# fujii-team/deComP

Hardware: AMD Instinct MI355X
Metric: nmf_mu_iterations_per_s (higher is better)
Workload: dtype f32; 1 GPU; nmf_mu l2 no-mask Y=65536x4096 k=256 fp32 (BASELINE configs[1]); rows_per_gpu=65536, parallelism=rows sharded x1, 1 all-reduce/step, loop=single-GPU dcp_nmf_mu_f32

## Files before the change

decomp_amd/_hip.py:

```python
import ctypes
import os
import threading

_HERE = os.path.dirname(os.path.abspath(__file__))
LIB_PATH = os.path.join(_HERE, 'lib', 'libdecomp_hip.so')

OK = 0
ERR_NAMES = {-1: 'DCP_ERR_INVALID', -2: 'DCP_ERR_HIP', -3: 'DCP_ERR_NOMEM',
             -4: 'DCP_ERR_INTERNAL', -5: 'DCP_ERR_UNSUPPORTED', -6: 'DCP_ERR_REF_TYPEERROR',
             -7: 'DCP_ERR_COMM'}
LIK_L2, LIK_KL, LIK_BETA = 0, 1, 2
PROF_NLABELS = 10
PROF_XUPDATE, PROF_STATS = 2, 4
LASSO_ISTA, LASSO_ACC_ISTA, LASSO_FISTA, LASSO_CD = 0, 1, 2, 3
LASSO_PARALLEL_CD, LASSO_ADMM = 4, 5
LASSO_OMP = 6
LASSO_POSITIVE = 0x100
ERR_REF_TYPEERROR = -6
ERR_COMM = -7
COMM_ID_BYTES = 128
ALLREDUCE_FN = ctypes.CFUNCTYPE(ctypes.c_int, ctypes.c_void_p, ctypes.c_int64, ctypes.c_int, ctypes.c_void_p, ctypes.c_void_p)

_c_int, _c_i64, _c_vp = ctypes.c_int, ctypes.c_int64, ctypes.c_void_p
_c_f32, _c_f64 = ctypes.c_float, ctypes.c_double
# ... 6 lines not shown
_P_INT, _P_F64 = _P(_c_int), _P(_c_f64)
_NFK = [_c_i64] * 3
_TM = [_c_i64] * 5 + [_c_int]
_TM_MC = [_c_i64] * 6 + [_c_int]
_MASKED = [_c_vp] * 3 + [_c_int, _c_vp, _c_vp] + _NFK

_FAMILIES = [
    ('dcp_create', None, [_P(_c_vp), _c_int]),
    ('dcp_destroy', None, [_c_vp]),
    ('dcp_set_stream', None, [_c_vp, _c_vp]),
    ('dcp_last_error_string', None, [_c_vp], ctypes.c_char_p),
    ('dcp_build_info', None, [], ctypes.c_char_p),
    ('dcp_comm_unique_id', None, [_c_vp, _c_i64]),
    ('dcp_comm_init', None, [_c_vp, _c_vp, _c_int, _c_int]),
    ('dcp_comm_destroy', None, [_c_vp]),
    ('dcp_comm_set_external', None, [_c_vp] * 3 + [_c_int, _c_int]),
    ('dcp_memcpy', None, [_c_vp] * 3 + [_c_i64]),
    ('dcp_comm_info', None, [_c_vp, _P_INT, _P_INT]),
    ('dcp_comm_allreduce_sum', _REALS, [_c_vp, _c_vp, _c_i64]),
    ('dcp_profile_enable', None, [_c_vp, _c_int]),
    ('dcp_profile_reset', None, [_c_vp]),
    ('dcp_profile_select', None, [_c_vp, ctypes.c_uint]),
    ('dcp_profile_read', None, [_c_vp, _c_int, _P_F64, _P(_c_i64)]),
    ('dcp_profile_label_name', None, [_c_int], ctypes.c_char_p),
    ('dcp_l2_normalize', _ALL, [_c_vp, _c_vp, _c_i64, _c_i64, _c_int]),
    ('dcp_l2_normalize_diff', _REALS, [_c_vp] * 4 + [_c_i64, _c_i64, _c_int, _P_F64]),
    ('dcp_count_negative', _REALS, [_c_vp, _c_vp, _c_i64, _P(_c_i64)]),
    ('dcp_gershgorin', _ALL, [_c_vp, _c_vp, _c_i64, _c_i64, _c_vp]),
    ('dcp_inv', _ALL, [_c_vp, _c_vp, _c_i64, _c_i64, _c_vp]),
    ('dcp_mu_quotient', _REALS, [_c_vp] * 4 + [_c_i64, _c_i64, _c_vp]),
    ('dcp_axpby', _REALS, [_c_vp, _c_i64, _c_f64, _c_vp, _c_f64, _c_vp]),
    ('dcp_gemm', _ALL, [_c_vp, _c_int] + [_c_vp] * 3 + _NFK + [_c_int, _c_int]),
    ('dcp_gemm_bf16x6', ('f32',), [_c_vp, _c_int] + [_c_vp] * 3 + _NFK + [_c_int]),
    ('dcp_set_f32_product_mode', None, [_c_vp, _c_int]),
    ('dcp_debug_tn_plain', None, [_c_int]),
    ('dcp_debug_gemm_route', None, [_c_int, _c_int] + [_c_i64] * 4 + [_c_int] * 5 + [_c_vp]),
    ('dcp_calib_read', ('f32',), [_c_vp, _c_vp, _c_i64, _c_i64, _c_int, _c_vp]),
    ('dcp_gather_rows_bytes', None, [_c_vp] * 3 + [_c_i64, _c_i64, _c_vp]),
    ('dcp_scatter_rows_bytes', None, [_c_vp] * 3 + [_c_i64, _c_i64, _c_vp]),
    ('dcp_dict_prefetch_rows_bytes', None, [_c_vp] * 3 + [_c_i64, _c_i64, _c_vp]),
    ('dcp_gather_rows', _ALL, [_c_vp] * 3 + [_c_i64, _c_i64, _c_vp]),
    ('dcp_nmf_mu', _REALS, [_c_vp] * 5 + _NFK + [_c_int, _REAL, _c_int, _P_INT, _P_REAL, _P_REAL]),
    ('dcp_nmf_mu_sharded', _REALS, [_c_vp] * 5 + _NFK + [_c_int, _REAL, _c_int, _P_INT, _P_REAL]),
    ('dcp_nmf_hals', _REALS, [_c_vp] * 4 + _NFK + [_REAL, _c_int, _P_INT, _P_REAL, _P_REAL]),
    ('dcp_nmf_hals_sharded', _REALS, [_c_vp] * 4 + _NFK + [_REAL, _c_int, _P_INT, _P_REAL]),
    ('dcp_nmf_emhals', _REALS, [_c_vp] * 5 + _NFK + [_REAL, _c_int, _P_INT, _P_REAL, _P_REAL]),
    ('dcp_nmf_emhals_sharded', _REALS, [_c_vp] * 5 + _NFK + [_REAL, _c_int, _P_INT, _P_REAL]),
    ('dcp_nmf_impute', _REALS, [_c_vp] * 5 + _NFK + [_c_vp]),
    ('dcp_nmf_hals_stats', _REALS, [_c_vp] * 5 + _NFK + [_c_vp]),
    ('dcp_nmf_hals_update', _REALS, [_c_vp] * 5 + _NFK + [_c_vp, _c_vp]),
    ('dcp_nn_cd_sweep', _REALS, [_c_vp] * 5 + [_c_i64, _c_i64, _c_int]),
    ('dcp_nmf_mu_stats_width', None, [_c_i64, _c_i64, _c_int, _c_int], _c_i64),
    ('dcp_nmf_mu_stats', _REALS, [_c_vp] * 6 + _NFK + [_c_int, _c_vp]),
    ('dcp_nmf_mask_bits_words', None, [_c_i64, _c_i64], _c_i64),
    ('dcp_nmf_mask_prepare', _REALS, [_c_vp] * 3 + [_c_i64, _c_i64, _c_vp, _c_vp, _P_INT]),
    ('dcp_nmf_mu_stats_prepared', _REALS, [_c_vp] * 7 + _NFK + [_c_int, _c_vp]),
    ('dcp_nmf_mu_update', _REALS, [_c_vp] * 4 + [_c_i64, _c_i64, _c_int, _c_int, _c_vp, _c_vp]),
    ('dcp_nmf_grads', _REALS, [_c_vp] * 5 + _NFK + [_c_int, _c_int, _c_vp, _c_vp]),
    ('dcp_nmf_grad_x', _REALS, [_c_vp] * 5 + _NFK + [_c_int, _c_vp, _c_vp]),
    ('dcp_nmf_gauss_logp', _REALS, [_c_vp] * 5 + _NFK + [_c_f64, _P_F64]),
    ('dcp_set_nmf_beta', None, [_c_vp, _c_f64]),
    ('dcp_set_nmf_penalty', None, [_c_vp, _c_f64, _c_f64]),
    ('dcp_nmf_beta_divergence', _REALS, [_c_vp] * 5 + _NFK + [_P_F64]),
    ('dcp_nmf_apply', _REALS, [_c_vp] * 4 + [_c_f64, _c_vp, _c_i64, _c_i64, _P_F64]),
    ('dcp_nmf_residual', _REALS, [_c_vp] * 5 + _NFK + [_P_F64]),
    ('dcp_lasso', _ALL, _MASKED + [_c_f64, _c_f64, _c_int, _c_int, _c_int, _P_INT]),
# ... 107 lines not shown
```

decomp_amd/csrc/gemm.hpp:

```cpp
#pragma once
#include <type_traits>

#include "epilogue.hpp"
#include "gemm_generic.hpp"
#include "gemm_mfma_bf16x6.hpp"
#include "gemm_mfma_f32.hpp"
#include "gemm_mfma_f64.hpp"
#include "reduce.hpp"
#include "scalar.hpp"

namespace dcp {

enum GemmForm { FORM_NT = 0, FORM_NN = 1, FORM_TN = 2 };
enum TileSel { TILE_AUTO = 0, TILE_LARGE = 1, TILE_SMALL = 2, TILE_HUGE = 3, TILE_SMALL_DEEP = 4, TILE_MID = 5 };

template <class T>
struct GemmArgs {
    const T* A = nullptr;
    long lda = 0;
    const T* B = nullptr;
    long ldb = 0;
    const T* B2 = nullptr;
    long ldb2 = 0;
    int n_b1 = 0;
// ... 459 lines not shown
enum { X6_NONE = -1, X6_LARGE = 0, X6_HUGE = 1 };
constexpr int kX6HugeTnMinK = 1024;

template <class T>
inline bool x6_huge_tn_shape(const GemmArgs<T>& a, int n1, int klen) {
    return std::is_same<T, float>::value && a.A2 == nullptr && a.M > 0 && a.N > 0 && a.K > 0 &&
           a.M % X6Huge::BM == 0 && n1 % X6Huge::BN == 0 && (a.N - n1) % X6Huge::BN == 0 && klen >= kX6HugeTnMinK &&
           pick_tier<FORM_TN>(a.M, a.N, a.K, a.tile, true, true) == TIER_LARGE;
}

template <class T>
inline bool plan_splits_x6_tn(GemmArgs<T>& a, int n1, int max_splits) {
    if (a.M <= 0 || a.N <= 0 || a.K <= 0 || a.M % X6Huge::BM || n1 % X6Huge::BN || (a.N - n1) % X6Huge::BN)
        return false;
    const long tiles = (long)(a.M / X6Huge::BM) * (n1 / X6Huge::BN + (a.N - n1) / X6Huge::BN);
    const long kblocks = ceil_div(a.K, 16);
    long smax = kblocks / 32;
    if (smax < 1) smax = 1;
    if (smax > max_splits) smax = max_splits;
    long s = 256 / tiles;
    if (s > smax) s = smax;
    if (s < 1) s = 1;
    const int klen = (int)(((kblocks + s - 1) / s) * 16);
    if (!x6_huge_tn_shape(a, n1, klen)) return false;
    a.split_planned = true;
    a.klen = klen;
    a.ksplits = ceil_div(a.K, klen);
    return true;
}

template <int FORM>
inline int x6_tier(const GemmArgs<float>& a) {
    if (FORM == FORM_NN) return X6_NONE;
    const int tier = pick_tier<FORM>(a.M, a.N, a.K, a.tile, a.split_planned, true);
    const GemmProblem p = fill_problem<FORM>(a);
    if (FORM == FORM_NT && tier == TIER_HUGE && x6_eligible<X6Huge>(p)) return X6_HUGE;
    if (FORM == FORM_TN && tier == TIER_LARGE && x6_huge_tn_shape(a, a.B2 != nullptr ? a.n_b1 : a.N, a.ksplits > 1 ? a.klen : a.K) &&
        x6_eligible<X6Huge>(p))
        return X6_HUGE;
    if ((tier == TIER_LARGE || (FORM == FORM_NT && (tier == TIER_MID || tier == TIER_HUGE))) &&
        x6_eligible<X6Large>(p))
        return X6_LARGE;
    return X6_NONE;
}

template <int FORM, class Epi>
inline hipError_t gemm_bf16x6(hipStream_t stream, const GemmArgs<float>& a, const Epi& epi) {
    constexpr int AL = (FORM == FORM_TN) ? XMAJOR : KMAJOR;
    constexpr int BL = (FORM == FORM_NT) ? KMAJOR : XMAJOR;
    if constexpr (FORM == FORM_NN) {
        return hipErrorInvalidValue;
    } else {
        const int t = x6_tier<FORM>(a);
        if (t == X6_HUGE) return launch_gemm_bf16x6<X6Huge, AL, BL, Epi>(stream, fill_problem<FORM>(a), epi);
        if (t == X6_LARGE) return launch_gemm_bf16x6<X6Large, AL, BL, Epi>(stream, fill_problem<FORM>(a), epi);
        return hipErrorInvalidValue;
    }
}

}
```

decomp_amd/csrc/gemm_mfma_bf16x6.hpp:

```cpp
#pragma once
#include "gemm_mfma_f32.hpp"
#include <type_traits>

namespace dcp {

typedef __bf16 x6_bf16x4 __attribute__((ext_vector_type(4)));
typedef __bf16 x6_bf16x8 __attribute__((ext_vector_type(8)));

template <int BM_, int BN_, int WM_, int WN_, int MINW_, int STAGES_>
struct X6Cfg {
    static constexpr int BM = BM_, BN = BN_, BK = 16, WM = WM_, WN = WN_, MINW = MINW_;
    static constexpr int NWAVES = (BM_ / WM_) * (BN_ / WN_);
    static constexpr int NTHREADS = 64 * NWAVES;
    static constexpr int STAGES = STAGES_;
};
typedef X6Cfg<256, 256, 64, 64, 1, 3> X6Huge;
typedef X6Cfg<128, 128, 64, 64, 2, 2> X6Large;

template <int ROWS>
struct X6Panel {
    static constexpr int PLANE_BYTES = ROWS * 32;
    static constexpr int BYTES = 3 * PLANE_BYTES;
};

__device__ __forceinline__ int x6_chunk(int r, int q) { return r * 32 + ((q ^ ((r >> 3) & 1)) << 4); }

__device__ __forceinline__ void x6_split(f32x4 a, x6_bf16x4& h, x6_bf16x4& m, x6_bf16x4& l) {
    h = __builtin_convertvector(a, x6_bf16x4);
    const f32x4 r1 = a - __builtin_convertvector(h, f32x4);
    m = __builtin_convertvector(r1, x6_bf16x4);
    const f32x4 r2 = r1 - __builtin_convertvector(m, f32x4);
    l = __builtin_convertvector(r2, x6_bf16x4);
}

template <int LAY, int ROWS, int NT, int G>
__device__ __forceinline__ void x6_gload(f32x4 (&r)[G], const float* __restrict__ p, long ld, int row0, int k0,
                                         int tid) {
    static_assert(G * NT * 4 == ROWS * 16, "panel must be a whole number of 4-value groups per thread");
#pragma unroll
    for (int i = 0; i < G; ++i) {
        const int idx = tid + i * NT;
        if (LAY == KMAJOR) {
            const int row = idx >> 2, kq = idx & 3;
            r[i] = *reinterpret_cast<const f32x4*>(p + (long)(row0 + row) * ld + (k0 + 4 * kq));
        } else {
            const int g = idx % (ROWS / 4), k = idx / (ROWS / 4);
            r[i] = *reinterpret_cast<const f32x4*>(p + (long)(k0 + k) * ld + (row0 + 4 * g));
        }
    }
}

template <int ROWS>
__device__ __forceinline__ int x6_granule(int k, int g) {
    static_assert(ROWS >= 128, "the XOR swizzle needs 32 granules per k row");
    return k * (ROWS * 2) + ((g ^ ((k & 3) << 3)) << 3);
}

template <int LAY, int ROWS, int NT, int G>
__device__ __forceinline__ void x6_lds_store(char* s, const f32x4 (&r)[G], int tid) {
#pragma unroll
    for (int i = 0; i < G; ++i) {
        const int idx = tid + i * NT;
        int off;
        if (LAY == KMAJOR) {
            const int row = idx >> 2, kq = idx & 3;
            off = x6_chunk(row, kq >> 1) + ((kq & 1) << 3);
        } else {
            off = x6_granule<ROWS>(idx / (ROWS / 4), idx % (ROWS / 4));
        }
        x6_bf16x4 h, m, l;
        x6_split(r[i], h, m, l);
        *reinterpret_cast<x6_bf16x4*>(s + off) = h;
        *reinterpret_cast<x6_bf16x4*>(s + X6Panel<ROWS>::PLANE_BYTES + off) = m;
        *reinterpret_cast<x6_bf16x4*>(s + 2 * X6Panel<ROWS>::PLANE_BYTES + off) = l;
    }
}

template <int LAY, int ROWS>
__device__ __forceinline__ int x6_frag_off(int r0, int lane) {
    const int l31 = lane & 31, h = lane >> 5;
    if (LAY == KMAJOR) return x6_chunk(r0 + l31, h);
    const int q = (lane >> 2) & 3, pq = lane & 3, gh = (lane >> 4) & 1;
    return x6_granule<ROWS>(8 * h + q, (r0 >> 2) + 4 * gh + pq);
}

template <int LAY, int ROWS>
__device__ __forceinline__ x6_bf16x8 x6_frag(const char* plane, int off) {
    if (LAY == KMAJOR) return *reinterpret_cast<const x6_bf16x8*>(plane + off);
    typedef short s16x4 __attribute__((ext_vector_type(4)));
    typedef __attribute__((address_space(3))) s16x4 lds_s16x4;
    const s16x4 lo = __builtin_amdgcn_ds_read_tr16_b64_v4i16((lds_s16x4*)(plane + off));
    const s16x4 hi = __builtin_amdgcn_ds_read_tr16_b64_v4i16((lds_s16x4*)(plane + off + 4 * ROWS * 2));
    return __builtin_bit_cast(x6_bf16x8, __builtin_shufflevector(lo, hi, 0, 1, 2, 3, 4, 5, 6, 7));
}

template <class E, class = void>
struct epi_den_tail { static constexpr bool value = false; };
template <class E>
struct epi_den_tail<E, decltype((void)E::kDenTail)> { static constexpr bool value = E::kDenTail; };

typedef float x6_f32x2 __attribute__((ext_vector_type(2)));

__device__ __forceinline__ int x6_den_xoff(int r, int q) { return r * 16 + ((q ^ ((r >> 2) & 3)) << 2); }

template <class Epi>
__device__ __forceinline__ void x6_den_tail(f32x16 (&num)[2][2], const Epi& epi, char* smem, int m0, int n0, int tid) {
    constexpr int XS = 128 * 16 * 4;
    constexpr int GS = 16 * 256 * 4;
    constexpr int DBUF = XS + GS;
    const int lane = tid & 63, wave = tid >> 6;
    const int wm = wave >> 2, wn = wave & 3;
    const int l31 = lane & 31, h = lane >> 5;
    const int nkd = epi.depth >> 4;

    const int pr = tid >> 3, k2 = tid & 7;
    const float* xsrc = epi.cur + (long)(m0 + (pr >> 5) * 64 + (pr & 31)) * epi.ld_cur + 2 * k2;
    const int xdst = (x6_den_xoff(pr, k2 >> 1) + 2 * (k2 & 1)) * 4;
// ... 120 lines not shown
    int mt, nt;
    if (p.mt_fast) {
        mt = t % p.tiles_m;
        nt = t / p.tiles_m;
    } else {
        nt = t % p.tiles_n;
        mt = t / p.tiles_n;
    }
    const int m0 = mt * BM;
    const int kbeg = split * p.klen;
    const int kend = min(p.K, kbeg + p.klen);
    const float* Bp = p.B;
    long ldb = p.ldb;
    int nB0 = nt * BN;
    int n0 = nB0;
    if (nt >= p.tiles_n1) {
        Bp = p.B2;
        ldb = p.ldb2;
        nB0 = (nt - p.tiles_n1) * BN;
        n0 = p.n_b1 + nB0;
    }

    f32x16 acc[TM][TN];
#pragma unroll
    for (int i = 0; i < TM; ++i)
#pragma unroll
        for (int j = 0; j < TN; ++j)
#pragma unroll
            for (int r = 0; r < 16; ++r) acc[i][j][r] = 0.0f;

    static_assert(TM == 2, "one panel's staging per 32-row A block");
    constexpr int STAGES = Cfg::STAGES;
    static_assert(STAGES == 2 || STAGES == 3, "two buffers and a boundary barrier, or a ring of three");
    f32x4 ra[GA], rb[GB];
    const int nkb = (kend - kbeg) / BK;
    if (nkb > 0) {
        x6_gload<ALAY, BM, NT>(ra, p.A, p.lda, m0, kbeg, tid);
        x6_gload<BLAY, BN, NT>(rb, Bp, ldb, nB0, kbeg, tid);
        x6_lds_store<ALAY, BM, NT>(x6_smem, ra, tid);
        x6_lds_store<BLAY, BN, NT>(x6_smem + X6Panel<BM>::BYTES, rb, tid);
        const int k1 = kbeg + min(1, nkb - 1) * BK;
        x6_gload<ALAY, BM, NT>(ra, p.A, p.lda, m0, k1, tid);
        x6_gload<BLAY, BN, NT>(rb, Bp, ldb, nB0, k1, tid);
        if constexpr (STAGES == 3) {
            x6_lds_store<ALAY, BM, NT>(x6_smem + BUF, ra, tid);
            x6_lds_store<BLAY, BN, NT>(x6_smem + BUF + X6Panel<BM>::BYTES, rb, tid);
            const int k2 = kbeg + min(2, nkb - 1) * BK;
            x6_gload<ALAY, BM, NT>(ra, p.A, p.lda, m0, k2, tid);
            x6_gload<BLAY, BN, NT>(rb, Bp, ldb, nB0, k2, tid);
        }
    }
    __syncthreads();

    int aoff[TM], boff[TN];
#pragma unroll
    for (int i = 0; i < TM; ++i) aoff[i] = x6_frag_off<ALAY, BM>(wm * WM + i * 32, lane);
#pragma unroll
    for (int j = 0; j < TN; ++j) boff[j] = x6_frag_off<BLAY, BN>(wn * WN + j * 32, lane);

    constexpr int STAGE_AFTER = 2;
    auto kblock = [&](int cur, int nxt_off, int knext, auto stage_tag, auto bar_tag) {
        constexpr bool STAGE = decltype(stage_tag)::value;
        constexpr bool BAR = decltype(bar_tag)::value;
        const char* sA = x6_smem + cur;
        const char* sB = sA + X6Panel<BM>::BYTES;
        char* nxt = x6_smem + nxt_off;
        x6_bf16x8 fb[3][TN];
#pragma unroll
        for (int pl = 0; pl < 3; ++pl)
#pragma unroll
            for (int j = 0; j < TN; ++j) fb[pl][j] = x6_frag<BLAY, BN>(sB + pl * PB, boff[j]);
        constexpr int TA[6] = {2, 0, 1, 1, 0, 0};
        constexpr int TB[6] = {0, 2, 1, 0, 1, 0};
        auto group = [&](auto i_tag) {
            constexpr int i = decltype(i_tag)::value;
            x6_bf16x8 fa[3];
#pragma unroll
            for (int pl = 0; pl < 3; ++pl) fa[pl] = x6_frag<ALAY, BM>(sA + pl * PA, aoff[i]);
            if constexpr (BAR && i == 1) {
                __builtin_amdgcn_sched_barrier(0);
                __syncthreads();
                __builtin_amdgcn_sched_barrier(0);
            }
            auto mfmas = [&](int t0, int t1) {
#pragma unroll
                for (int tt = t0; tt < t1; ++tt)
#pragma unroll
                    for (int j = 0; j < TN; ++j)
                        acc[i][j] =
                            __builtin_amdgcn_mfma_f32_32x32x16_bf16(fa[TA[tt]], fb[TB[tt]][j], acc[i][j], 0, 0, 0);
            };
            if constexpr (STAGE) {
                mfmas(0, STAGE_AFTER);
                __builtin_amdgcn_sched_barrier(0);
                if constexpr (i == 0) {
                    x6_lds_store<ALAY, BM, NT>(nxt, ra, tid);
                    x6_gload<ALAY, BM, NT>(ra, p.A, p.lda, m0, knext, tid);
                } else {
                    x6_lds_store<BLAY, BN, NT>(nxt + X6Panel<BM>::BYTES, rb, tid);
                    x6_gload<BLAY, BN, NT>(rb, Bp, ldb, nB0, knext, tid);
                }
                __builtin_amdgcn_sched_barrier(0);
                mfmas(STAGE_AFTER, 6);
            } else {
                mfmas(0, 6);
            }
            __builtin_amdgcn_sched_barrier(0);
        };
        group(std::integral_constant<int, 0>{});
        group(std::integral_constant<int, 1>{});
    };
    if constexpr (STAGES == 2) {
        for (int kb = 0; kb + 1 < nkb; ++kb) {
            const int cur = (kb & 1) * BUF;
            kblock(cur, cur ^ BUF, kbeg + min(kb + 2, nkb - 1) * BK, std::true_type{}, std::false_type{});
            __syncthreads();
        }
        if (nkb > 0) kblock(((nkb - 1) & 1) * BUF, 0, 0, std::false_type{}, std::false_type{});
    } else {
        int b0 = 0, b1 = BUF, b2 = 2 * BUF;
        for (int kb = 0; kb + 2 < nkb; ++kb) {
            kblock(b0, b2, kbeg + min(kb + 3, nkb - 1) * BK, std::true_type{}, std::true_type{});
            const int t0 = b0;
            b0 = b1;
            b1 = b2;
            b2 = t0;
        }
        if (nkb > 1) kblock(b0, 0, 0, std::false_type{}, std::true_type{});
        if (nkb > 0) kblock(nkb > 1 ? b1 : b0, 0, 0, std::false_type{}, std::false_type{});
    }

    if constexpr (epi_den_tail<Epi>::value) {
        static_assert(BM == 256 && BN == 256 && NT == 1024 && STAGES == 3 && ALAY == KMAJOR && BLAY == KMAJOR,
                      "the denominator tail is laid out for the 256 x 256 NT tile");
        x6_den_tail(acc, epi, x6_smem, m0, n0, tid);
    } else if constexpr (epi_vec4<Epi>::value) {
        const int tq = l31 & 3, col0 = (l31 & ~3);
#pragma unroll
        for (int i = 0; i < TM; ++i)
#pragma unroll
            for (int j = 0; j < TN; ++j)
#pragma unroll
                for (int g = 0; g < 4; ++g) {
                    f32x4 x;
#pragma unroll
                    for (int e = 0; e < 4; ++e) x[e] = acc[i][j][4 * g + e];
                    const f32x4 y = quad_transpose(x, tq);
                    epi.vec4(m0 + wm * WM + i * 32 + 8 * g + 4 * h + tq, n0 + wn * WN + j * 32 + col0, y, split);
                }
    } else {
#pragma unroll
        for (int i = 0; i < TM; ++i)
#pragma unroll
            for (int j = 0; j < TN; ++j) {
                const int col = n0 + wn * WN + j * 32 + l31;
#pragma unroll
                for (int r = 0; r < 16; ++r) {
                    const int row = m0 + wm * WM + i * 32 + (r & 3) + 8 * (r >> 2) + 4 * h;
                    epi(row, col, acc[i][j][r], split);
                }
            }
    }
}

template <class Epi>
inline bool x6_epi_ok(const Epi& epi) {
    if constexpr (epi_vec4<Epi>::value) return epi.vec_ok();
    else return true;
}

template <class Cfg>
inline bool x6_eligible(const GemmProblem& p) {
    auto al16 = [](const void* q) { return (reinterpret_cast<uintptr_t>(q) & 15) == 0; };
    const int n1 = p.B2 != nullptr ? p.n_b1 : p.N;
    bool ok = p.M > 0 && p.N > 0 && p.K > 0 && (p.M % Cfg::BM) == 0 && (n1 % Cfg::BN) == 0 &&
              ((p.N - n1) % Cfg::BN) == 0 && (p.K % 16) == 0 && p.A2 == nullptr && (p.lda % 4) == 0 &&
              (p.ldb % 4) == 0 && al16(p.A) && al16(p.B);
    if (p.B2 != nullptr) ok = ok && (p.ldb2 % 4) == 0 && al16(p.B2);
    if (p.ksplits > 1) ok = ok && (p.klen % 16) == 0 && p.klen > 0;
    return ok;
}

template <class Cfg, int ALAY, int BLAY, class Epi>
inline hipError_t launch_gemm_bf16x6(hipStream_t stream, GemmProblem p, const Epi& epi) {
    if (!x6_eligible<Cfg>(p) || !x6_epi_ok(epi)) return hipErrorInvalidValue;
    if constexpr (epi_den_tail<Epi>::value) {
        if (p.ksplits > 1 || p.B2 != nullptr || epi.depth < 48 || (epi.depth % 16) != 0) return hipErrorInvalidValue;
    }
    if (p.B2 == nullptr) p.n_b1 = p.N;
    p.m_a1 = p.M;
    p.tiles_m1 = p.tiles_m = p.M / Cfg::BM;
    p.tiles_n1 = p.n_b1 / Cfg::BN;
    p.tiles_n = p.tiles_n1 + (p.N - p.n_b1) / Cfg::BN;
    if (p.ksplits < 1) p.ksplits = 1;
    if (p.ksplits == 1) p.klen = p.K;
    p.vec_epi = epi_vec4<Epi>::value ? 1 : 0;
    p.al_mask = 0;
    const int grid = p.tiles_m * p.tiles_n * p.ksplits;
    if (grid <= 0) return hipSuccess;
    constexpr int lds_bytes = Cfg::STAGES * (X6Panel<Cfg::BM>::BYTES + X6Panel<Cfg::BN>::BYTES);
    const void* fn = reinterpret_cast<const void*>(&gemm_bf16x6_kernel<Cfg, ALAY, BLAY, Epi>);
    if constexpr (lds_bytes > 65536) {
        static DynLdsRaised raised;
        std::atomic<bool>& done = raised.on_current_device();
        if (!done) {
            hipError_t e = hipFuncSetAttribute(fn, hipFuncAttributeMaxDynamicSharedMemorySize, lds_bytes);
            if (e != hipSuccess) return e;
            done = true;
        }
    }
    hipLaunchKernelGGL((gemm_bf16x6_kernel<Cfg, ALAY, BLAY, Epi>), dim3(grid), dim3(Cfg::NTHREADS), lds_bytes,
                       stream, p, epi);
    return hipGetLastError();
}

}
```

decomp_amd/csrc/util.hip:

```cpp
#include "abi.hpp"
#include "comm.hpp"
#include "gemm.hpp"
#include "handle.hpp"
#include "kernels_small.hpp"
#include <new>

#define DCP_STR2(x) #x
#define DCP_STR(x) DCP_STR2(x)

using namespace dcp;

namespace {

template <class T>
int l2_normalize_api(dcp_handle* h, T* U, int64_t K, int64_t F, int strict) {
    if (!h) return DCP_ERR_INVALID;
    if (!U) return fail(h, DCP_ERR_INVALID, "null array pointer");
    if (K < 0 || F < 0) return fail(h, DCP_ERR_INVALID, "negative size");
    if (K == 0 || F == 0) return DCP_OK;
    DCP_HIP_OK(h, hipSetDevice(h->device));
    hipLaunchKernelGGL((row_normalize_kernel<T>), dim3((unsigned)K), dim3(256), 0, h->stream,
                       (const T*)U, (long)F, (long)F, strict, (const T*)nullptr, 0L, U, (long)F,
                       (real_t<T>*)nullptr);
    DCP_HIP_OK(h, hipGetLastError());
// ... 473 lines not shown
        h->prof_cnt[i] = 0;
    }
    return DCP_OK;
}

int dcp_profile_read(dcp_handle* h, int label, double* total_ms, int64_t* count) {
    if (!h) return DCP_ERR_INVALID;
    if (label < 0 || label >= DCP_PROF_NLABELS || !total_ms || !count)
        return fail(h, DCP_ERR_INVALID, "bad profile label or null output");
    DCP_TRY(prof_fold(h));
    *total_ms = h->prof_ms[label];
    *count = h->prof_cnt[label];
    return DCP_OK;
}

const char* dcp_profile_label_name(int label) {
    static const char* names[DCP_PROF_NLABELS] = {"gram",  "x_neg",     "x_update", "forward", "stats",
                                                  "stats_sum", "d_update", "d_norm",  "misc", "exchange"};
    return (label >= 0 && label < DCP_PROF_NLABELS) ? names[label] : "?";
}

const char* dcp_last_error_string(dcp_handle* h) { return h ? h->err.c_str() : "null handle"; }

const char* dcp_build_info(void) {
    return "libdecomp_hip: gfx950, fp32 MFMA 32x32x2 + fp64 MFMA 16x16x4 GEMM cores, HIP " DCP_STR(HIP_VERSION_MAJOR) "." DCP_STR(HIP_VERSION_MINOR);
}

int dcp_count_negative_f32(dcp_handle* h, const float* x, int64_t n, int64_t* count) {
    return count_negative_api<float>(h, x, n, count);
}
int dcp_count_negative_f64(dcp_handle* h, const double* x, int64_t n, int64_t* count) {
    return count_negative_api<double>(h, x, n, count);
}
int dcp_gemm_bf16x6_f32(dcp_handle* h, int form, const float* A, const float* B, float* C, int64_t M, int64_t N,
                        int64_t K, int ksplits) {
    if (!h) return DCP_ERR_INVALID;
    if (!A || !B || !C) return fail(h, DCP_ERR_INVALID, "null array pointer");
    if (M <= 0 || N <= 0 || K <= 0 || M > INT32_MAX || N > INT32_MAX || K > INT32_MAX)
        return fail(h, DCP_ERR_INVALID, "bad sizes");
    if (form != FORM_NT && form != FORM_TN) return fail(h, DCP_ERR_INVALID, "bf16x6: form must be 0 (NT) or 2 (TN)");
    DCP_HIP_OK(h, hipSetDevice(h->device));
    GemmArgs<float> a;
    a.A = A; a.B = B; a.M = (int)M; a.N = (int)N; a.K = (int)K;
    a.lda = (form == FORM_TN) ? M : K;
    a.ldb = (form == FORM_NT) ? K : N;
    float* slabs = nullptr;
    if (ksplits > 1) {
        const long kblocks = (K + 15) / 16;
        const long s = ksplits > kblocks ? kblocks : ksplits;
        a.klen = (int)(((kblocks + s - 1) / s) * 16);
        a.ksplits = (int)((K + a.klen - 1) / a.klen);
        a.split_planned = true;
        DCP_TRY(ws_lay_out(h, [&](WsLayout& w) { w.take(slabs, (size_t)a.ksplits * M * N); }));
    }
    const bool ok = (form == FORM_NT) ? x6_tier<FORM_NT>(a) != X6_NONE : x6_tier<FORM_TN>(a) != X6_NONE;
    if (!ok) return fail(h, DCP_ERR_INVALID, "bf16x6: no split-bf16 kernel for this shape (tiles, alignment)");
    hipError_t e;
    if (slabs) {
        EpiSlab<float> epi{slabs, (long)N, (long)M * N};
        e = (form == FORM_NT) ? gemm_bf16x6<FORM_NT>(h->stream, a, epi) : gemm_bf16x6<FORM_TN>(h->stream, a, epi);
        if (e != hipSuccess) return fail(h, DCP_ERR_HIP, hipGetErrorString(e));
        launch_reduce_slabs_scalar<float>(h->stream, slabs, (long)(M * N), a.ksplits, (long)(M * N), C);
        DCP_HIP_OK(h, hipGetLastError());
    } else {
        EpiStore<float> epi{C, (long)N};
        e = (form == FORM_NT) ? gemm_bf16x6<FORM_NT>(h->stream, a, epi) : gemm_bf16x6<FORM_TN>(h->stream, a, epi);
        if (e != hipSuccess) return fail(h, DCP_ERR_HIP, hipGetErrorString(e));
    }
    return DCP_OK;
}
int dcp_set_f32_product_mode(dcp_handle* h, int mode) {
    if (!h) return DCP_ERR_INVALID;
    const int prev = h->f32_product_mode;
    if (mode > 1) return fail(h, DCP_ERR_INVALID, "f32 product mode must be 0 (bf16x6) or 1 (fp32)");
    if (mode >= 0) h->f32_product_mode = mode;
    return prev;
}

int dcp_dict_prefetch_rows_bytes(dcp_handle* h, const void* in, const int64_t* index, int64_t rows,
                                 int64_t row_bytes, void* out) {
    if (!h) return DCP_ERR_INVALID;
    if (rows < 0 || row_bytes < 0) return dcp::fail(h, DCP_ERR_INVALID, "negative size");
    if (rows > 0 && row_bytes > 0 && (!in || !index || !out)) return dcp::fail(h, DCP_ERR_INVALID, "null pointer");
    h->pf_in = in;
    h->pf_index = index;
    h->pf_out = out;
    h->pf_rows = rows;
    h->pf_row_bytes = row_bytes;
    return DCP_OK;
}

int dcp_gather_rows_bytes(dcp_handle* h, const void* in, const int64_t* index, int64_t rows,
                          int64_t row_bytes, void* out) {
    if (h && !index) return dcp::fail(h, DCP_ERR_INVALID, "null index");
    return move_rows(h, in, index, out, nullptr, rows, row_bytes);
}

int dcp_scatter_rows_bytes(dcp_handle* h, const void* in, const int64_t* index, int64_t rows,
                           int64_t row_bytes, void* out) {
    if (h && !index) return dcp::fail(h, DCP_ERR_INVALID, "null index");
    return move_rows(h, in, nullptr, out, index, rows, row_bytes);
}

// ... 22 lines not shown
```

include/decomp_hip.h:

```cpp
#ifndef DECOMP_HIP_H
#define DECOMP_HIP_H

#include <stdint.h>

#ifdef __cplusplus
extern "C" {
#endif

typedef struct dcp_handle dcp_handle;

enum {
    DCP_OK = 0,
    DCP_ERR_INVALID = -1,
    DCP_ERR_HIP = -2,
    DCP_ERR_NOMEM = -3,
    DCP_ERR_INTERNAL = -4,
    DCP_ERR_UNSUPPORTED = -5,
    DCP_ERR_REF_TYPEERROR = -6,
    DCP_ERR_COMM = -7
};

enum { DCP_LIK_L2 = 0, DCP_LIK_KL = 1, DCP_LIK_BETA = 2 };

enum { DCP_LASSO_ISTA = 0, DCP_LASSO_ACC_ISTA = 1, DCP_LASSO_FISTA = 2, DCP_LASSO_CD = 3,
// ... 36 lines not shown
int dcp_profile_reset(dcp_handle* h);
int dcp_profile_read(dcp_handle* h, int label, double* total_ms, int64_t* count);
const char* dcp_profile_label_name(int label);

int dcp_l2_normalize_f32(dcp_handle* h, float* U, int64_t K, int64_t F, int strict);
int dcp_l2_normalize_f64(dcp_handle* h, double* U, int64_t K, int64_t F, int strict);
int dcp_l2_normalize_c64(dcp_handle* h, void* U, int64_t K, int64_t F, int strict);
int dcp_l2_normalize_c128(dcp_handle* h, void* U, int64_t K, int64_t F, int strict);

int dcp_count_negative_f32(dcp_handle* h, const float* x, int64_t n, int64_t* count);
int dcp_count_negative_f64(dcp_handle* h, const double* x, int64_t n, int64_t* count);

int dcp_gershgorin_f32(dcp_handle* h, const float* X, int64_t batch, int64_t n, float* out);
int dcp_gershgorin_f64(dcp_handle* h, const double* X, int64_t batch, int64_t n, double* out);
int dcp_gershgorin_c64(dcp_handle* h, const void* X, int64_t batch, int64_t n, float* out);
int dcp_gershgorin_c128(dcp_handle* h, const void* X, int64_t batch, int64_t n, double* out);

int dcp_inv_f32(dcp_handle* h, const float* X, int64_t batch, int64_t n, float* out);
int dcp_inv_f64(dcp_handle* h, const double* X, int64_t batch, int64_t n, double* out);
int dcp_inv_c64(dcp_handle* h, const void* X, int64_t batch, int64_t n, void* out);
int dcp_inv_c128(dcp_handle* h, const void* X, int64_t batch, int64_t n, void* out);

int dcp_gemm_f32(dcp_handle* h, int form, const float* A, const float* B, float* C,
                 int64_t M, int64_t N, int64_t K, int ksplits, int tile);
int dcp_gemm_f64(dcp_handle* h, int form, const double* A, const double* B, double* C,
                 int64_t M, int64_t N, int64_t K, int ksplits, int tile);
int dcp_gemm_c64(dcp_handle* h, int form, const void* A, const void* B, void* C,
                 int64_t M, int64_t N, int64_t K, int ksplits, int tile);
int dcp_gemm_c128(dcp_handle* h, int form, const void* A, const void* B, void* C,
                  int64_t M, int64_t N, int64_t K, int ksplits, int tile);

int dcp_gemm_bf16x6_f32(dcp_handle* h, int form, const float* A, const float* B, float* C,
                        int64_t M, int64_t N, int64_t K, int ksplits);

int dcp_set_f32_product_mode(dcp_handle* h, int mode);

int dcp_debug_tn_plain(int on);

int dcp_debug_gemm_route(int dtype, int form, int64_t M, int64_t N, int64_t K, int64_t n_b1, int tile, int flags,
                         int target_wgs, int max_splits, int min_blocks, int32_t* out);

int dcp_calib_read_f32(dcp_handle* h, const float* p, int64_t rows, int64_t cols, int pattern,
                       float* out);

int dcp_nmf_mu_f32(dcp_handle* h, const float* Y, const float* mask, float* X, float* D,
                   int64_t N, int64_t F, int64_t K, int likelihood, float tol, int maxiter,
                   int* it_out, float* last_maxdiff, float* resid_trace);
int dcp_nmf_mu_f64(dcp_handle* h, const double* Y, const double* mask, double* X, double* D,
                   int64_t N, int64_t F, int64_t K, int likelihood, double tol, int maxiter,
                   int* it_out, double* last_maxdiff, double* resid_trace);

int dcp_nmf_hals_f32(dcp_handle* h, const float* Y, float* X, float* D, int64_t N, int64_t F, int64_t K,
                     float tol, int maxiter, int* it_out, float* last_maxdiff, float* resid_trace);
int dcp_nmf_hals_f64(dcp_handle* h, const double* Y, double* X, double* D, int64_t N, int64_t F, int64_t K,
                     double tol, int maxiter, int* it_out, double* last_maxdiff, double* resid_trace);
int dcp_nmf_hals_sharded_f32(dcp_handle* h, const float* Y, float* X, float* D, int64_t N, int64_t F, int64_t K,
                             float tol, int maxiter, int* it_out, float* last_maxdiff);
int dcp_nmf_hals_sharded_f64(dcp_handle* h, const double* Y, double* X, double* D, int64_t N, int64_t F, int64_t K,
                             double tol, int maxiter, int* it_out, double* last_maxdiff);
int dcp_nmf_hals_stats_f32(dcp_handle* h, const float* Y, const float* X, float* X_out, const float* D, int64_t N,
                           int64_t F, int64_t K, float* stats);
int dcp_nmf_hals_stats_f64(dcp_handle* h, const double* Y, const double* X, double* X_out, const double* D,
                           int64_t N, int64_t F, int64_t K, double* stats);
int dcp_nmf_hals_update_f32(dcp_handle* h, const float* stats, const float* D, float* D_new, float* X, int64_t N,
                            int64_t F, int64_t K, float* maxdiff_dev, float* maxdiff_next);
int dcp_nmf_hals_update_f64(dcp_handle* h, const double* stats, const double* D, double* D_new, double* X,
// ... 385 lines not shown
```

Baseline: 690.1 iterations/s.

## Preload bf16x6 LDS fragments across k-blocks and use scalar-base global loads

For the three-stage bf16x6 MFMA GEMM, the main loop now reads the next k-block's A/B fragments from LDS in small pieces between MFMA groups and moves the in-block barrier to sit between them. This is meant to hide LDS read latency behind matrix math instead of reloading all fragments at the start of each block. Global loads now use a scalar base pointer plus 32-bit per-lane offsets to cut address arithmetic, with an eligibility check that the offsets fit in 32 bits. It also adds a segmented-B API entry, a tier query helper and optional s_memtime timing stamps behind a compile flag, and it raises register pressure by keeping fragments live across blocks.

```diff
diff --git a/decomp_amd/_hip.py b/decomp_amd/_hip.py
--- a/decomp_amd/_hip.py
+++ b/decomp_amd/_hip.py
@@ -62,6 +62,8 @@
     ('dcp_axpby', _REALS, [_c_vp, _c_i64, _c_f64, _c_vp, _c_f64, _c_vp]),
     ('dcp_gemm', _ALL, [_c_vp, _c_int] + [_c_vp] * 3 + _NFK + [_c_int, _c_int]),
     ('dcp_gemm_bf16x6', ('f32',), [_c_vp, _c_int] + [_c_vp] * 3 + _NFK + [_c_int]),
+    ('dcp_gemm_bf16x6_seg', ('f32',), [_c_vp, _c_int] + [_c_vp] * 4 + [_c_i64] * 4 + [_c_int]),
+    ('dcp_gemm_bf16x6_tier', None, [_c_int] + [_c_i64] * 4 + [_c_int]),
     ('dcp_set_f32_product_mode', None, [_c_vp, _c_int]),
     ('dcp_debug_tn_plain', None, [_c_int]),
     ('dcp_debug_gemm_route', None, [_c_int, _c_int] + [_c_i64] * 4 + [_c_int] * 5 + [_c_vp]),
diff --git a/decomp_amd/csrc/gemm.hpp b/decomp_amd/csrc/gemm.hpp
--- a/decomp_amd/csrc/gemm.hpp
+++ b/decomp_amd/csrc/gemm.hpp
@@ -515,14 +515,15 @@
 template <int FORM>
 inline int x6_tier(const GemmArgs<float>& a) {
     if (FORM == FORM_NN) return X6_NONE;
+    constexpr int AL = (FORM == FORM_TN) ? XMAJOR : KMAJOR, BL = (FORM == FORM_NT) ? KMAJOR : XMAJOR;
     const int tier = pick_tier<FORM>(a.M, a.N, a.K, a.tile, a.split_planned, true);
     const GemmProblem p = fill_problem<FORM>(a);
-    if (FORM == FORM_NT && tier == TIER_HUGE && x6_eligible<X6Huge>(p)) return X6_HUGE;
+    if (FORM == FORM_NT && tier == TIER_HUGE && x6_eligible<X6Huge, AL, BL>(p)) return X6_HUGE;
     if (FORM == FORM_TN && tier == TIER_LARGE && x6_huge_tn_shape(a, a.B2 != nullptr ? a.n_b1 : a.N, a.ksplits > 1 ? a.klen : a.K) &&
-        x6_eligible<X6Huge>(p))
+        x6_eligible<X6Huge, AL, BL>(p))
         return X6_HUGE;
     if ((tier == TIER_LARGE || (FORM == FORM_NT && (tier == TIER_MID || tier == TIER_HUGE))) &&
-        x6_eligible<X6Large>(p))
+        x6_eligible<X6Large, AL, BL>(p))
         return X6_LARGE;
     return X6_NONE;
 }
diff --git a/decomp_amd/csrc/gemm_mfma_bf16x6.hpp b/decomp_amd/csrc/gemm_mfma_bf16x6.hpp
--- a/decomp_amd/csrc/gemm_mfma_bf16x6.hpp
+++ b/decomp_amd/csrc/gemm_mfma_bf16x6.hpp
@@ -3,6 +3,16 @@
 #include <type_traits>
 
 namespace dcp {
+
+#ifdef DCP_X6_STAMPS
+static __device__ unsigned long long x6_stamp_buf[16 * 8];
+#define X6_STAMP(t)                                                                         \
+    do {                                                                                    \
+        __builtin_amdgcn_sched_barrier(0);                                                  \
+        asm volatile("s_memtime %0\n\ts_waitcnt lgkmcnt(0)" : "=s"(t) : : "memory");        \
+        __builtin_amdgcn_sched_barrier(0);                                                  \
+    } while (0)
+#endif
 
 typedef __bf16 x6_bf16x4 __attribute__((ext_vector_type(4)));
 typedef __bf16 x6_bf16x8 __attribute__((ext_vector_type(8)));
@@ -33,20 +43,37 @@
     l = __builtin_convertvector(r2, x6_bf16x4);
 }
 
-template <int LAY, int ROWS, int NT, int G>
+template <int LAY, int ROWS, int NT, bool SBASE, int G>
 __device__ __forceinline__ void x6_gload(f32x4 (&r)[G], const float* __restrict__ p, long ld, int row0, int k0,
                                          int tid) {
     static_assert(G * NT * 4 == ROWS * 16, "panel must be a whole number of 4-value groups per thread");
+    if constexpr (!SBASE) {
+#pragma unroll
+        for (int i = 0; i < G; ++i) {
+            const int idx = tid + i * NT;
+            if (LAY == KMAJOR) {
+                const int row = idx >> 2, kq = idx & 3;
+                r[i] = *reinterpret_cast<const f32x4*>(p + (long)(row0 + row) * ld + (k0 + 4 * kq));
+            } else {
+                const int g = idx % (ROWS / 4), k = idx / (ROWS / 4);
+                r[i] = *reinterpret_cast<const f32x4*>(p + (long)(k0 + k) * ld + (row0 + 4 * g));
+            }
+        }
+        return;
+    }
+    typedef const __attribute__((address_space(1))) char* gchar_ptr;
+    typedef const __attribute__((address_space(1))) f32x4* gf32x4_ptr;
+    gchar_ptr base = (gchar_ptr)(p + (LAY == KMAJOR ? (long)row0 * ld + k0 : (long)k0 * ld + row0));
+    asm("" : "+s"(base));
 #pragma unroll
     for (int i = 0; i < G; ++i) {
         const int idx = tid + i * NT;
-        if (LAY == KMAJOR) {
-            const int row = idx >> 2, kq = idx & 3;
-            r[i] = *reinterpret_cast<const f32x4*>(p + (long)(row0 + row) * ld + (k0 + 4 * kq));
-        } else {
-            const int g = idx % (ROWS / 4), k = idx / (ROWS / 4);
-            r[i] = *reinterpret_cast<const f32x4*>(p + (long)(k0 + k) * ld + (row0 + 4 * g));
-        }
+        unsigned off;
+        if (LAY == KMAJOR) off = (unsigned)(idx >> 2) * (unsigned)ld + 4u * (idx & 3);
+        else off = (unsigned)(idx / (ROWS / 4)) * (unsigned)ld + 4u * (idx % (ROWS / 4));
+        off *= 4u;
+        asm("" : "+v"(off));
+        r[i] = *(gf32x4_ptr)(base + off);
     }
 }
 
@@ -83,6 +110,9 @@
     const int q = (lane >> 2) & 3, pq = lane & 3, gh = (lane >> 4) & 1;
     return x6_granule<ROWS>(8 * h + q, (r0 >> 2) + 4 * gh + pq);
 }
+
+template <int LAY>
+__device__ __forceinline__ int x6_frag_next32(int off) { return LAY == KMAJOR ? off + 32 * 32 : off ^ 64; }
 
 template <int LAY, int ROWS>
 __device__ __forceinline__ x6_bf16x8 x6_frag(const char* plane, int off) {
@@ -269,55 +299,97 @@
     static_assert(TM == 2, "one panel's staging per 32-row A block");
     constexpr int STAGES = Cfg::STAGES;
     static_assert(STAGES == 2 || STAGES == 3, "two buffers and a boundary barrier, or a ring of three");
+    constexpr bool REFILL = STAGES == 3;
     f32x4 ra[GA], rb[GB];
     const int nkb = (kend - kbeg) / BK;
     if (nkb > 0) {
-        x6_gload<ALAY, BM, NT>(ra, p.A, p.lda, m0, kbeg, tid);
-        x6_gload<BLAY, BN, NT>(rb, Bp, ldb, nB0, kbeg, tid);
+        x6_gload<ALAY, BM, NT, REFILL>(ra, p.A, p.lda, m0, kbeg, tid);
+        x6_gload<BLAY, BN, NT, REFILL>(rb, Bp, ldb, nB0, kbeg, tid);
         x6_lds_store<ALAY, BM, NT>(x6_smem, ra, tid);
         x6_lds_store<BLAY, BN, NT>(x6_smem + X6Panel<BM>::BYTES, rb, tid);
         const int k1 = kbeg + min(1, nkb - 1) * BK;
-        x6_gload<ALAY, BM, NT>(ra, p.A, p.lda, m0, k1, tid);
-        x6_gload<BLAY, BN, NT>(rb, Bp, ldb, nB0, k1, tid);
+        x6_gload<ALAY, BM, NT, REFILL>(ra, p.A, p.lda, m0, k1, tid);
+        x6_gload<BLAY, BN, NT, REFILL>(rb, Bp, ldb, nB0, k1, tid);
         if constexpr (STAGES == 3) {
             x6_lds_store<ALAY, BM, NT>(x6_smem + BUF, ra, tid);
             x6_lds_store<BLAY, BN, NT>(x6_smem + BUF + X6Panel<BM>::BYTES, rb, tid);
             const int k2 = kbeg + min(2, nkb - 1) * BK;
-            x6_gload<ALAY, BM, NT>(ra, p.A, p.lda, m0, k2, tid);
-            x6_gload<BLAY, BN, NT>(rb, Bp, ldb, nB0, k2, tid);
+            x6_gload<ALAY, BM, NT, REFILL>(ra, p.A, p.lda, m0, k2, tid);
+            x6_gload<BLAY, BN, NT, REFILL>(rb, Bp, ldb, nB0, k2, tid);
         }
     }
     __syncthreads();
 
-    int aoff[TM], boff[TN];
-#pragma unroll
-    for (int i = 0; i < TM; ++i) aoff[i] = x6_frag_off<ALAY, BM>(wm * WM + i * 32, lane);
-#pragma unroll
-    for (int j = 0; j < TN; ++j) boff[j] = x6_frag_off<BLAY, BN>(wn * WN + j * 32, lane);
+    static_assert(WM == 64 && WN == 64 && TN == 2, "x6_frag_next32: two 32-row blocks per 64-row wave tile");
+    const int aoff = x6_frag_off<ALAY, BM>(wm * WM, lane), boff = x6_frag_off<BLAY, BN>(wn * WN, lane);
+    int aoff2[TM], boff2[TN];
+#pragma unroll
+    for (int i = 0; i < TM; ++i) aoff2[i] = REFILL ? 0 : x6_frag_off<ALAY, BM>(wm * WM + i * 32, lane);
+#pragma unroll
+    for (int j = 0; j < TN; ++j) boff2[j] = REFILL ? 0 : x6_frag_off<BLAY, BN>(wn * WN + j * 32, lane);
 
     constexpr int STAGE_AFTER = 2;
-    auto kblock = [&](int cur, int nxt_off, int knext, auto stage_tag, auto bar_tag) {
+    constexpr int TA[6] = {2, 0, 1, 1, 0, 0};
+    constexpr int TB[6] = {0, 2, 1, 0, 1, 0};
+    x6_bf16x8 fa[3], fb[3][TN];
+    auto afrag = [&](int off, int pl) { return x6_frag<ALAY, BM>(x6_smem + pl * PA, off); };
+    auto bfrag = [&](int off, int pl, int j) {
+        return x6_frag<BLAY, BN>(x6_smem + X6Panel<BM>::BYTES + pl * PB, j ? x6_frag_next32<BLAY>(off) : off);
+    };
+    auto ring_off = [](int buf, int off) {
+        int o = buf + off;
+        asm("" : "+v"(o));
+        return o;
+    };
+#ifdef DCP_X6_STAMPS
+    unsigned long long st_t0 = 0, st_t1 = 0, st_t2 = 0, st_t3 = 0, st_a = 0, st_b = 0, st_first = 0, st_last = 0;
+    unsigned long long st_cost = 0;
+    unsigned st_n = 0;
+    X6_STAMP(st_t1);
+    X6_STAMP(st_t0);
+    st_cost = st_t0 - st_t1;
+#endif
+    if constexpr (REFILL) {
+#pragma unroll
+        for (int pl = 2; pl >= 0; --pl) {
+#pragma unroll
+            for (int j = 0; j < TN; ++j) fb[pl][j] = bfrag(boff, pl, j);
+            fa[pl] = afrag(aoff, pl);
+        }
+    }
+    auto kblock = [&](int cur, int nxt_off, int knext, int nb, auto stage_tag, auto bar_tag, auto next_tag) {
         constexpr bool STAGE = decltype(stage_tag)::value;
         constexpr bool BAR = decltype(bar_tag)::value;
-        const char* sA = x6_smem + cur;
-        const char* sB = sA + X6Panel<BM>::BYTES;
+        constexpr bool NEXT = decltype(next_tag)::value;
+        static_assert(REFILL || (!BAR && !NEXT), "the barrier inside the block and the early reads need the ring");
         char* nxt = x6_smem + nxt_off;
-        x6_bf16x8 fb[3][TN];
-#pragma unroll
-        for (int pl = 0; pl < 3; ++pl)
-#pragma unroll
-            for (int j = 0; j < TN; ++j) fb[pl][j] = x6_frag<BLAY, BN>(sB + pl * PB, boff[j]);
-        constexpr int TA[6] = {2, 0, 1, 1, 0, 0};
-        constexpr int TB[6] = {0, 2, 1, 0, 1, 0};
+#ifdef DCP_X6_STAMPS
+        if constexpr (BAR) {
+            X6_STAMP(st_t1);
+            st_a += st_t1 - st_t0;
+            if (st_n == 0) st_first = st_t0;
+            st_last = st_t0;
+            ++st_n;
+        }
+#endif
+        if constexpr (!REFILL) {
+#pragma unroll
+            for (int pl = 0; pl < 3; ++pl)
+#pragma unroll
+                for (int j = 0; j < TN; ++j)
+                    fb[pl][j] = x6_frag<BLAY, BN>(x6_smem + cur + X6Panel<BM>::BYTES + pl * PB, boff2[j]);
+        }
         auto group = [&](auto i_tag) {
             constexpr int i = decltype(i_tag)::value;
-            x6_bf16x8 fa[3];
-#pragma unroll
-            for (int pl = 0; pl < 3; ++pl) fa[pl] = x6_frag<ALAY, BM>(sA + pl * PA, aoff[i]);
-            if constexpr (BAR && i == 1) {
-                __builtin_amdgcn_sched_barrier(0);
-                __syncthreads();
-                __builtin_amdgcn_sched_barrier(0);
+            if constexpr (!REFILL) {
+#pragma unroll
+                for (int pl = 0; pl < 3; ++pl) fa[pl] = x6_frag<ALAY, BM>(x6_smem + cur + pl * PA, aoff2[i]);
+            }
+            int roa = 0, rob = 0;
+            if constexpr (REFILL && i == 0) roa = x6_frag_next32<ALAY>(ring_off(cur, aoff));
+            if constexpr (REFILL && i == 1 && NEXT) {
+                roa = ring_off(nb, aoff);
+                rob = ring_off(nb, boff);
             }
             auto mfmas = [&](int t0, int t1) {
 #pragma unroll
@@ -327,20 +399,64 @@
                         acc[i][j] =
                             __builtin_amdgcn_mfma_f32_32x32x16_bf16(fa[TA[tt]], fb[TB[tt]][j], acc[i][j], 0, 0, 0);
             };
+            auto refill_a = [&](int pl) {
+                if constexpr (i == 0 || NEXT) fa[pl] = afrag(roa, pl);
+            };
+            auto refill_b = [&](int pl) {
+                if constexpr (i == 1 && NEXT) {
+#pragma unroll
+                    for (int j = 0; j < TN; ++j) fb[pl][j] = bfrag(rob, pl, j);
+                }
+            };
+            mfmas(0, 1);
+            if constexpr (REFILL) {
+                __builtin_amdgcn_sched_barrier(0);
+                if constexpr (BAR && i == 1) {
+                    __syncthreads();
+                    __builtin_amdgcn_sched_barrier(0);
+#ifdef DCP_X6_STAMPS
+                    X6_STAMP(st_t3);
+                    st_b += st_t3 - st_t2;
+#endif
+                }
+                refill_a(2);
+                __builtin_amdgcn_sched_barrier(0);
+            }
+            mfmas(1, STAGE_AFTER);
+            if constexpr (REFILL) {
+                __builtin_amdgcn_sched_barrier(0);
+                refill_b(2);
+            }
             if constexpr (STAGE) {
-                mfmas(0, STAGE_AFTER);
                 __builtin_amdgcn_sched_barrier(0);
                 if constexpr (i == 0) {
                     x6_lds_store<ALAY, BM, NT>(nxt, ra, tid);
-                    x6_gload<ALAY, BM, NT>(ra, p.A, p.lda, m0, knext, tid);
+                    x6_gload<ALAY, BM, NT, REFILL>(ra, p.A, p.lda, m0, knext, tid);
                 } else {
                     x6_lds_store<BLAY, BN, NT>(nxt + X6Panel<BM>::BYTES, rb, tid);
-                    x6_gload<BLAY, BN, NT>(rb, Bp, ldb, nB0, knext, tid);
+                    x6_gload<BLAY, BN, NT, REFILL>(rb, Bp, ldb, nB0, knext, tid);
                 }
-                __builtin_amdgcn_sched_barrier(0);
+            }
+            if constexpr (REFILL || STAGE) __builtin_amdgcn_sched_barrier(0);
+            if constexpr (REFILL) {
+                mfmas(STAGE_AFTER, 4);
+                __builtin_amdgcn_sched_barrier(0);
+                refill_a(1);
+                __builtin_amdgcn_sched_barrier(0);
+                mfmas(4, 5);
+                __builtin_amdgcn_sched_barrier(0);
+                refill_b(1);
+                __builtin_amdgcn_sched_barrier(0);
+                mfmas(5, 6);
+#ifdef DCP_X6_STAMPS
+                if constexpr (BAR && i == 0) X6_STAMP(st_t2);
+                if constexpr (BAR && i == 1) X6_STAMP(st_t0);
+#endif
+                __builtin_amdgcn_sched_barrier(0);
+                refill_b(0);
+                refill_a(0);
+            } else {
                 mfmas(STAGE_AFTER, 6);
-            } else {
-                mfmas(0, 6);
             }
             __builtin_amdgcn_sched_barrier(0);
         };
@@ -350,22 +466,36 @@
     if constexpr (STAGES == 2) {
         for (int kb = 0; kb + 1 < nkb; ++kb) {
             const int cur = (kb & 1) * BUF;
-            kblock(cur, cur ^ BUF, kbeg + min(kb + 2, nkb - 1) * BK, std::true_type{}, std::false_type{});
+            kblock(cur, cur ^ BUF, kbeg + min(kb + 2, nkb - 1) * BK, 0, std::true_type{}, std::false_type{},
+                   std::false_type{});
             __syncthreads();
         }
-        if (nkb > 0) kblock(((nkb - 1) & 1) * BUF, 0, 0, std::false_type{}, std::false_type{});
+        if (nkb > 0)
+            kblock(((nkb - 1) & 1) * BUF, 0, 0, 0, std::false_type{}, std::false_type{}, std::false_type{});
     } else {
         int b0 = 0, b1 = BUF, b2 = 2 * BUF;
         for (int kb = 0; kb + 2 < nkb; ++kb) {
-            kblock(b0, b2, kbeg + min(kb + 3, nkb - 1) * BK, std::true_type{}, std::true_type{});
+            kblock(b0, b2, kbeg + min(kb + 3, nkb - 1) * BK, b1, std::true_type{}, std::true_type{},
+                   std::true_type{});
             const int t0 = b0;
             b0 = b1;
             b1 = b2;
             b2 = t0;
         }
-        if (nkb > 1) kblock(b0, 0, 0, std::false_type{}, std::true_type{});
-        if (nkb > 0) kblock(nkb > 1 ? b1 : b0, 0, 0, std::false_type{}, std::false_type{});
-    }
+        if (nkb > 1) kblock(b0, 0, 0, b1, std::false_type{}, std::true_type{}, std::true_type{});
+        if (nkb > 0) kblock(nkb > 1 ? b1 : b0, 0, 0, 0, std::false_type{}, std::false_type{}, std::false_type{});
+    }
+
+#ifdef DCP_X6_STAMPS
+    if (blockIdx.x == 0 && lane == 0) {
+        unsigned long long* o = x6_stamp_buf + wave * 8;
+        o[0] = st_a;
+        o[1] = st_b;
+        o[2] = st_last - st_first;
+        o[3] = st_n;
+        o[4] = st_cost;
+    }
+#endif
 
     if constexpr (epi_den_tail<Epi>::value) {
         static_assert(BM == 256 && BN == 256 && NT == 1024 && STAGES == 3 && ALAY == KMAJOR && BLAY == KMAJOR,
@@ -406,21 +536,25 @@
     else return true;
 }
 
-template <class Cfg>
+template <class Cfg, int ALAY, int BLAY>
 inline bool x6_eligible(const GemmProblem& p) {
     auto al16 = [](const void* q) { return (reinterpret_cast<uintptr_t>(q) & 15) == 0; };
     const int n1 = p.B2 != nullptr ? p.n_b1 : p.N;
     bool ok = p.M > 0 && p.N > 0 && p.K > 0 && (p.M % Cfg::BM) == 0 && (n1 % Cfg::BN) == 0 &&
               ((p.N - n1) % Cfg::BN) == 0 && (p.K % 16) == 0 && p.A2 == nullptr && (p.lda % 4) == 0 &&
               (p.ldb % 4) == 0 && al16(p.A) && al16(p.B);
-    if (p.B2 != nullptr) ok = ok && (p.ldb2 % 4) == 0 && al16(p.B2);
+    auto off32 = [](int lay, int rows, long ld) {
+        return Cfg::STAGES != 3 || ((lay == KMAJOR ? (rows - 1) * ld + 16 : 15 * ld + rows) * 4 < (1L << 32));
+    };
+    ok = ok && off32(ALAY, Cfg::BM, p.lda) && off32(BLAY, Cfg::BN, p.ldb);
+    if (p.B2 != nullptr) ok = ok && (p.ldb2 % 4) == 0 && al16(p.B2) && off32(BLAY, Cfg::BN, p.ldb2);
     if (p.ksplits > 1) ok = ok && (p.klen % 16) == 0 && p.klen > 0;
     return ok;
 }
 
 template <class Cfg, int ALAY, int BLAY, class Epi>
 inline hipError_t launch_gemm_bf16x6(hipStream_t stream, GemmProblem p, const Epi& epi) {
-    if (!x6_eligible<Cfg>(p) || !x6_epi_ok(epi)) return hipErrorInvalidValue;
+    if (!x6_eligible<Cfg, ALAY, BLAY>(p) || !x6_epi_ok(epi)) return hipErrorInvalidValue;
     if constexpr (epi_den_tail<Epi>::value) {
         if (p.ksplits > 1 || p.B2 != nullptr || epi.depth < 48 || (epi.depth % 16) != 0) return hipErrorInvalidValue;
     }
diff --git a/decomp_amd/csrc/util.hip b/decomp_amd/csrc/util.hip
--- a/decomp_amd/csrc/util.hip
+++ b/decomp_amd/csrc/util.hip
@@ -529,25 +529,47 @@
 int dcp_count_negative_f64(dcp_handle* h, const double* x, int64_t n, int64_t* count) {
     return count_negative_api<double>(h, x, n, count);
 }
-int dcp_gemm_bf16x6_f32(dcp_handle* h, int form, const float* A, const float* B, float* C, int64_t M, int64_t N,
-                        int64_t K, int ksplits) {
-    if (!h) return DCP_ERR_INVALID;
-    if (!A || !B || !C) return fail(h, DCP_ERR_INVALID, "null array pointer");
-    if (M <= 0 || N <= 0 || K <= 0 || M > INT32_MAX || N > INT32_MAX || K > INT32_MAX)
-        return fail(h, DCP_ERR_INVALID, "bad sizes");
-    if (form != FORM_NT && form != FORM_TN) return fail(h, DCP_ERR_INVALID, "bf16x6: form must be 0 (NT) or 2 (TN)");
-    DCP_HIP_OK(h, hipSetDevice(h->device));
-    GemmArgs<float> a;
+static void bf16x6_hook_args(GemmArgs<float>& a, int form, const float* A, const float* B, const float* B2, int64_t M,
+                             int64_t N, int64_t n_b1, int64_t K, int ksplits) {
     a.A = A; a.B = B; a.M = (int)M; a.N = (int)N; a.K = (int)K;
     a.lda = (form == FORM_TN) ? M : K;
-    a.ldb = (form == FORM_NT) ? K : N;
-    float* slabs = nullptr;
+    a.ldb = (form == FORM_NT) ? K : n_b1;
+    if (B2) {
+        a.B2 = B2; a.n_b1 = (int)n_b1;
+        a.ldb2 = (form == FORM_NT) ? K : N - n_b1;
+    }
     if (ksplits > 1) {
         const long kblocks = (K + 15) / 16;
         const long s = ksplits > kblocks ? kblocks : ksplits;
         a.klen = (int)(((kblocks + s - 1) / s) * 16);
         a.ksplits = (int)((K + a.klen - 1) / a.klen);
         a.split_planned = true;
+    }
+}
+
+int dcp_gemm_bf16x6_tier(int form, int64_t M, int64_t N, int64_t n_b1, int64_t K, int ksplits) {
+    if ((form != FORM_NT && form != FORM_TN) || M <= 0 || N <= 0 || K <= 0 || n_b1 <= 0 || n_b1 > N || M > INT32_MAX ||
+        N > INT32_MAX || K > INT32_MAX)
+        return X6_NONE;
+    alignas(16) static const float aligned[4] = {0, 0, 0, 0};
+    GemmArgs<float> a;
+    bf16x6_hook_args(a, form, aligned, aligned, n_b1 < N ? aligned : nullptr, M, N, n_b1, K, ksplits);
+    return (form == FORM_NT) ? x6_tier<FORM_NT>(a) : x6_tier<FORM_TN>(a);
+}
+
+int dcp_gemm_bf16x6_seg_f32(dcp_handle* h, int form, const float* A, const float* B, const float* B2, float* C,
+                            int64_t M, int64_t N, int64_t n_b1, int64_t K, int ksplits) {
+    if (!h) return DCP_ERR_INVALID;
+    if (!A || !B || !C) return fail(h, DCP_ERR_INVALID, "null array pointer");
+    if (M <= 0 || N <= 0 || K <= 0 || M > INT32_MAX || N > INT32_MAX || K > INT32_MAX)
+        return fail(h, DCP_ERR_INVALID, "bad sizes");
+    if (B2 ? (n_b1 <= 0 || n_b1 >= N) : n_b1 != N) return fail(h, DCP_ERR_INVALID, "bf16x6: bad first segment width");
+    if (form != FORM_NT && form != FORM_TN) return fail(h, DCP_ERR_INVALID, "bf16x6: form must be 0 (NT) or 2 (TN)");
+    DCP_HIP_OK(h, hipSetDevice(h->device));
+    GemmArgs<float> a;
+    bf16x6_hook_args(a, form, A, B, B2, M, N, n_b1, K, ksplits);
+    float* slabs = nullptr;
+    if (ksplits > 1) {
         DCP_TRY(ws_lay_out(h, [&](WsLayout& w) { w.take(slabs, (size_t)a.ksplits * M * N); }));
     }
     const bool ok = (form == FORM_NT) ? x6_tier<FORM_NT>(a) != X6_NONE : x6_tier<FORM_TN>(a) != X6_NONE;
@@ -566,6 +588,18 @@
     }
     return DCP_OK;
 }
+int dcp_gemm_bf16x6_f32(dcp_handle* h, int form, const float* A, const float* B, float* C, int64_t M, int64_t N,
+                        int64_t K, int ksplits) {
+    return dcp_gemm_bf16x6_seg_f32(h, form, A, B, nullptr, C, M, N, N, K, ksplits);
+}
+#ifdef DCP_X6_STAMPS
+extern "C" int dcp_x6_stamps_read(unsigned long long* out) {
+    if (hipDeviceSynchronize() != hipSuccess) return DCP_ERR_HIP;
+    return hipMemcpyFromSymbol(out, HIP_SYMBOL(dcp::x6_stamp_buf), sizeof(dcp::x6_stamp_buf)) == hipSuccess
+               ? DCP_OK
+               : DCP_ERR_HIP;
+}
+#endif
 int dcp_set_f32_product_mode(dcp_handle* h, int mode) {
     if (!h) return DCP_ERR_INVALID;
     const int prev = h->f32_product_mode;
diff --git a/include/decomp_hip.h b/include/decomp_hip.h
--- a/include/decomp_hip.h
+++ b/include/decomp_hip.h
@@ -92,6 +92,10 @@
 
 int dcp_gemm_bf16x6_f32(dcp_handle* h, int form, const float* A, const float* B, float* C,
                         int64_t M, int64_t N, int64_t K, int ksplits);
+
+int dcp_gemm_bf16x6_seg_f32(dcp_handle* h, int form, const float* A, const float* B, const float* B2, float* C,
+                            int64_t M, int64_t N, int64_t n_b1, int64_t K, int ksplits);
+int dcp_gemm_bf16x6_tier(int form, int64_t M, int64_t N, int64_t n_b1, int64_t K, int ksplits);
 
 int dcp_set_f32_product_mode(dcp_handle* h, int mode);
 
```

Result: faster. 710.3 iterations/s, median of 6 (+2.9%).
